# voitta-ai/voitta-rag

Measured on AMD Instinct MI355X. Metric: chunks indexed/sec + p50 top-10 query latency @1M-chunk corpus, 1/8 MI355X, higher is better.
Workload: dtype f16 (f16 MFMA operands, f32 accumulate; softmax, LayerNorm statistics and pooling in f32; the residual stream between layers is stored as f16 (LayerNorm is applied inside the GEMM epilogues from f32 row sums); measured |1-cos| = 1.5e-6 vs the f64 oracle on THIS code path at this scale — 2300 sequenc

## Files before the change

voitta_rag_amd/csrc/encoder.hip:

```cpp

#include "engine_internal.h"

#include <map>
#include <tuple>

#include <algorithm>
#include <cmath>

namespace vr {

using f32x4 = __attribute__((ext_vector_type(4))) float;
using f32x16 = __attribute__((ext_vector_type(16))) float;

struct SplitWeight {
  _Float16* hi = nullptr;
  _Float16* lo = nullptr;
  float unscale = 1.0f;
};

struct LayerWeights {
  float *wqkv, *bqkv, *wo, *bo, *ln1g, *ln1b, *w1, *b1, *w2, *b2, *ln2g, *ln2b;
  SplitWeight s_qkv, s_o, s_1, s_2;
  SplitWeight s_qkv_f{}, s_1_f{};
  float *cs_qkv = nullptr, *c_qkv = nullptr, *cs_1 = nullptr, *c_1 = nullptr;
  SplitWeight s_qkv_p{}, s_1_p{};
  float *bqkv_p = nullptr, *b1_p = nullptr;
  SplitWeight s_1_fp{};
  float *cs_1_p = nullptr, *c_1_p = nullptr;
  float *qn = nullptr, *kn = nullptr;
};

constexpr int kMaxHeadStages = 4;
struct HeadStage {
  int kind, in_dim, out_dim, act;
  float eps;
  const float *w, *b;
};
struct HeadParams {
  int n_stages;
  HeadStage st[kMaxHeadStages];
};

struct Encoder {
  vr_bert_desc d{};
  float *word = nullptr, *pos = nullptr, *type = nullptr, *lng = nullptr, *lnb = nullptr;
  std::vector<LayerWeights> layers;
  std::vector<float*> owned;
  int64_t ws_tokens = 0;
  float *x = nullptr, *qkv = nullptr, *ctx = nullptr, *tmp = nullptr, *ffn = nullptr;
  float* xs = nullptr;
  float* lnstat = nullptr;
  float* lnpart = nullptr;
  float* glu = nullptr;
  float2* rope = nullptr;
  float2* rope_local = nullptr;
  float* bias = nullptr;
  int bias_radius = 0;
  float* slopes = nullptr;
  bool has_head = false;
  HeadParams head{};
  int out_dim = 0;
  DevArray<float> pooled;
  int causal = 0;
  int dh = 0, attn = 0, qk_norm = 0;
  int window_stream_from = 0;
  float* posidx = nullptr;
  bool fuse = true;
  DevArray<int32_t> ids, cu, seg;
  DevArray<int32_t> span_tok, span_seq;
  std::vector<int32_t> span_seq_host;
  DevArray<int32_t> sem_off, sem_start, sem_idx, sem_seq_chunks, sem_seq_base, sem_counter;
  DevArray<float> sem_sums, sem_dist, sem_rows;
  DevArray<float> out;
  float *pool_w = nullptr, *pool_b = nullptr, *cls_w = nullptr, *cls_b = nullptr;
  float *head_ln_g = nullptr, *head_ln_b = nullptr;
  DevArray<float> rows;
  DevArray<float> skinny_ws;
  struct GraphKey {
    int T, n_seq, max_len;
    const void *ids, *cu, *seg, *out;
    const void *span_tok = nullptr, *span_seq = nullptr;
    int n_spans = 0;
    const void* pooled = nullptr;
    bool operator<(const GraphKey& o) const {
      return std::tie(T, n_seq, max_len, ids, cu, seg, out, span_tok, span_seq, n_spans, pooled) <
             std::tie(o.T, o.n_seq, o.max_len, o.ids, o.cu, o.seg, o.out, o.span_tok, o.span_seq, o.n_spans, o.pooled);
    }
  };
  struct GraphEntry {
    int seen = 0;
    bool bad = false;
    hipGraphExec_t exec = nullptr;
  };
  std::map<GraphKey, GraphEntry> graphs;
};

static void invalidate_graphs(Encoder* enc) {
  for (auto& kv : enc->graphs)
    if (kv.second.exec) (void)hipGraphExecDestroy(kv.second.exec);
  enc->graphs.clear();
}


__device__ __forceinline__ float wave_sum(float v) {
#pragma unroll
  for (int off = 32; off >= 1; off >>= 1) v += __shfl_xor(v, off);
  return v;
}

constexpr int kMaxPairs = 8;

using half_t = _Float16;
using f16x8 = __attribute__((ext_vector_type(8))) _Float16;

__device__ __forceinline__ void split_f16(float v, half_t& hi, half_t& lo) {
  v = fminf(fmaxf(v, -65504.0f), 65504.0f);
  hi = static_cast<half_t>(v);
  lo = static_cast<half_t>(v - static_cast<float>(hi));
}
// ... 877 lines not shown
  for (int t = 0; t < kHeadTiles; ++t) {
    const int col = (wave + 4 * t) * 16 + r;
    if (col < ocols)
#pragma unroll
      for (int i = 0; i < 4; ++i)
        if (p0 + 4 * q + i < n) out[static_cast<int64_t>(p0 + 4 * q + i) * ostride + col] = act[t][i];
  }
}

static int head_lda(const HeadParams& hp) {
  int k = 0;
  for (int s = 0; s < hp.n_stages; ++s)
    if (hp.st[s].kind == VR_HEAD_DENSE) k = std::max(k, hp.st[s].in_dim);
  return k + 4;
}
static size_t head_lds_bytes(int lda) { return (64 + 16 * static_cast<size_t>(lda)) * sizeof(float); }
constexpr int kMaxHeadWidth = 1024;

static int out_width(const Encoder* enc) { return enc->has_head ? enc->out_dim : enc->d.hidden; }

__global__ __launch_bounds__(256) void gather_first_rows_kernel(const float4* __restrict__ src,
                                                                const int32_t* __restrict__ cu, int seq0,
                                                                int tok_base, int n, int T, int row_f4,
                                                                float4* __restrict__ dst) {
  const int lane = threadIdx.x & 63;
  const int i = blockIdx.x * 4 + (threadIdx.x >> 6);
  if (i >= n) return;
  const int t = min(cu[seq0 + i] - tok_base, T - 1);
  for (int c = lane; c < row_f4; c += 64) dst[static_cast<int64_t>(i) * row_f4 + c] = src[static_cast<int64_t>(t) * row_f4 + c];
}

__global__ __launch_bounds__(256) void gather_first_rows_ln_kernel(const float* __restrict__ pre,
                                                                   const float2* __restrict__ stat,
                                                                   const float* __restrict__ g,
                                                                   const float* __restrict__ b,
                                                                   const int32_t* __restrict__ cu, int seq0,
                                                                   int tok_base, int n, int T, int H,
                                                                   float* __restrict__ dst) {
  const int lane = threadIdx.x & 63;
  const int i = blockIdx.x * 4 + (threadIdx.x >> 6);
  if (i >= n) return;
  const int t = min(cu[seq0 + i] - tok_base, T - 1);
  const float2 st = stat[t];
  for (int c = lane; c < H; c += 64)
    dst[static_cast<int64_t>(i) * H + c] = ln_apply(pre[static_cast<int64_t>(t) * H + c], st.x, st.y, g[c], b[c]);
}

__global__ __launch_bounds__(256) void gather_first_rows_ln16_kernel(const half_t* __restrict__ pre,
                                                                     const float2* __restrict__ stat,
                                                                     const float* __restrict__ g,
                                                                     const float* __restrict__ b,
                                                                     const int32_t* __restrict__ cu, int seq0,
                                                                     int tok_base, int n, int T, int H,
                                                                     float* __restrict__ dst) {
  const int lane = threadIdx.x & 63;
  const int i = blockIdx.x * 4 + (threadIdx.x >> 6);
  if (i >= n) return;
  const int t = min(cu[seq0 + i] - tok_base, T - 1);
  const float2 st = stat[t];
  for (int c = lane; c < H; c += 64)
    dst[static_cast<int64_t>(i) * H + c] =
        ln_apply(static_cast<float>(pre[static_cast<int64_t>(t) * H + c]), st.x, st.y, g[c], b[c]);
}


__device__ __forceinline__ void load8(const float* p, float (&v)[8]) {
  const float4 a = *reinterpret_cast<const float4*>(p), b = *reinterpret_cast<const float4*>(p + 4);
  v[0] = a.x, v[1] = a.y, v[2] = a.z, v[3] = a.w, v[4] = b.x, v[5] = b.y, v[6] = b.z, v[7] = b.w;
}
__device__ __forceinline__ void load8(const half_t* p, float (&v)[8]) {
  const f16x8 h = *reinterpret_cast<const f16x8*>(p);
#pragma unroll
  for (int k = 0; k < 8; ++k) v[k] = static_cast<float>(h[k]);
}
__device__ __forceinline__ void store8(float* p, const float (&v)[8]) {
  *reinterpret_cast<float4*>(p) = make_float4(v[0], v[1], v[2], v[3]);
  *reinterpret_cast<float4*>(p + 4) = make_float4(v[4], v[5], v[6], v[7]);
}
__device__ __forceinline__ void store8(half_t* p, const float (&v)[8]) {
  f16x8 h;
#pragma unroll
  for (int k = 0; k < 8; ++k) h[k] = static_cast<half_t>(fminf(fmaxf(v[k], -65504.0f), 65504.0f));
  *reinterpret_cast<f16x8*>(p) = h;
}

template <typename T>
__global__ __launch_bounds__(256) void rope_kernel(T* __restrict__ qkv, const int32_t* __restrict__ pos, int Tn, int H,
                                                   int dh, const float2* __restrict__ table) {
  const int lane = threadIdx.x & 63;
  const int t = blockIdx.x * 4 + (threadIdx.x >> 6);
  if (t >= Tn) return;
  const int half = dh >> 1;
  const int groups = half >> 3;
  const int per_third = (H / dh) * groups;
  T* row = qkv + static_cast<int64_t>(t) * 3 * H;
  const float2* cs_row = table + static_cast<int64_t>(pos[t]) * (H >> 1);
  for (int c = lane; c < 2 * per_third; c += 64) {
    const int third = c >= per_third ? 1 : 0;
    const int w = c - third * per_third;
    const int head = w / groups, i8 = (w - head * groups) << 3;
    T* at = row + third * H + head * dh + i8;
    float a[8], b[8], cs0[8], cs1[8];
    load8(at, a);
    load8(at + half, b);
    load8(reinterpret_cast<const float*>(cs_row + i8), cs0);
    load8(reinterpret_cast<const float*>(cs_row + i8 + 4), cs1);
    float ra[8], rb[8];
#pragma unroll
    for (int k = 0; k < 8; ++k) {
      const float co = k < 4 ? cs0[2 * k] : cs1[2 * k - 8], si = k < 4 ? cs0[2 * k + 1] : cs1[2 * k - 7];
      ra[k] = a[k] * co - b[k] * si;
      rb[k] = b[k] * co + a[k] * si;
    }
    store8(at, ra);
    store8(at + half, rb);
// ... 2620 lines not shown
        mx = fmaxf(mx, __shfl_xor(mx, 16));
        mx = fmaxf(mx, __shfl_xor(mx, 32));
        const float m_raw = fmaxf(m[i], mx);
        const float m_new = WIN || CAUSAL ? softmax_base(m_raw) : m_raw;
        const float alpha = __builtin_amdgcn_exp2f(m[i] - m_new);
        float psum = 0.0f;
#pragma unroll
        for (int t = 0; t < 4; ++t)
#pragma unroll
          for (int r = 0; r < 4; ++r) {
            const float p = __builtin_amdgcn_exp2f(st[i][t][r] - m_new);
            psum += p;
            pb[i][t >> 1][(t & 1) * 4 + r] = static_cast<half_t>(p);
          }
        l[i] = l[i] * alpha + psum;
        m[i] = m_raw;
#pragma unroll
        for (int s = 0; s < NS; ++s) o[i][s] *= alpha;
      }
#pragma unroll
      for (int u = 0; u < 2; ++u)
#pragma unroll
        for (int s = 0; s < NS; ++s) {
          const half_t* vb = sV + (32 * u + 4 * g) * LDK + tr_row + ((2 * s + (tr_p >> 1)) ^ tr_sw) * 8 + tr_in;
          const s16x4 lo = __builtin_amdgcn_ds_read_tr16_b64_v4i16((__attribute__((address_space(3))) s16x4*)(vb));
          const s16x4 hi = __builtin_amdgcn_ds_read_tr16_b64_v4i16((__attribute__((address_space(3))) s16x4*)(vb + 16 * LDK));
          f16x8 vf;
          *reinterpret_cast<s16x4*>(&vf) = lo;
          *(reinterpret_cast<s16x4*>(&vf) + 1) = hi;
          o[0][s] = __builtin_amdgcn_mfma_f32_16x16x32_f16(vf, pb[0][u], o[0][s], 0, 0, 0);
          if (two) o[1][s] = __builtin_amdgcn_mfma_f32_16x16x32_f16(vf, pb[1][u], o[1][s], 0, 0, 0);
        }
    }
    if (more) write(kt + 64, kr, vr, att_tiles + 2 * (buf ^ 1) * TILE, att_tiles + (2 * (buf ^ 1) + 1) * TILE);
    __syncthreads();
  }
  if (!active) return;
#pragma unroll
  for (int i = 0; i < 2; ++i) {
    float li = l[i];
    li += __shfl_xor(li, 16);
    li += __shfl_xor(li, 32);
    const int q_tok = qw + 16 * i + qi;
    if (q_tok < len && (i == 0 || two)) {
      const float inv = 1.0f / li;
      const int64_t off = static_cast<int64_t>(t0 + q_tok) * H + head * DH + 4 * g;
#pragma unroll
      for (int s = 0; s < NS; ++s) {
        half_t h[4];
#pragma unroll
        for (int r = 0; r < 4; ++r) h[r] = static_cast<half_t>(fminf(fmaxf(o[i][s][r] * inv, -65504.0f), 65504.0f));
        *reinterpret_cast<uint2*>(ctx_h + off + 16 * s) = *reinterpret_cast<const uint2*>(h);
      }
    }
  }
}


static int dev_alloc_copy(vr_engine* e, Encoder* enc, const void* src, size_t n_floats, int mem, float** out) {
  float* p = nullptr;
  VR_HIP(hipMalloc(reinterpret_cast<void**>(&p), n_floats * sizeof(float)));
  enc->owned.push_back(p);
  if (src)
    VR_HIP(hipMemcpyAsync(p, src, n_floats * sizeof(float),
                          mem == VR_MEM_HOST ? hipMemcpyHostToDevice : hipMemcpyDeviceToDevice, e->stream));
  *out = p;
  return 0;
}

__global__ void ln_finalize_kernel(const float2* __restrict__ part, int T, int segs, int H, float eps,
                                   float2* __restrict__ stat) {
  const int t = blockIdx.x * blockDim.x + threadIdx.x;
  if (t >= T) return;
  float s1 = 0.0f, s2 = 0.0f;
  for (int i = 0; i < segs; ++i) {
    const float2 p = part[static_cast<int64_t>(t) * segs + i];
    s1 += p.x;
    s2 += p.y;
  }
  const float mean = s1 / static_cast<float>(H);
  const float var = fmaxf(s2 / static_cast<float>(H) - mean * mean, 0.0f);
  stat[t] = make_float2(mean, 1.0f / sqrtf(var + eps));
}

__global__ void scale_cols_kernel(const float* __restrict__ w, const float* __restrict__ g, int64_t n, int K,
                                  float* __restrict__ out) {
  const int64_t i = static_cast<int64_t>(blockIdx.x) * blockDim.x + threadIdx.x;
  if (i < n) out[i] = w[i] * g[i % K];
}

__global__ __launch_bounds__(256) void fold_vectors_kernel(const half_t* __restrict__ wq, float unscale,
                                                           const float* __restrict__ w, const float* __restrict__ b,
                                                           const float* __restrict__ bias, int N, int K,
                                                           float* __restrict__ colsum, float* __restrict__ c) {
  const int lane = threadIdx.x & 63;
  const int n = blockIdx.x * 4 + (threadIdx.x >> 6);
  if (n >= N) return;
  double sq = 0.0, sc = 0.0;
  for (int k = lane; k < K; k += 64) {
    sq += static_cast<double>(static_cast<float>(wq[static_cast<int64_t>(n) * K + k]));
    sc += static_cast<double>(w[static_cast<int64_t>(n) * K + k]) * static_cast<double>(b[k]);
  }
#pragma unroll
  for (int off = 32; off >= 1; off >>= 1) {
    sq += __shfl_xor(sq, off);
    sc += __shfl_xor(sc, off);
// ... 139 lines not shown
           "position table are not implemented", d->position);
  VR_CHECK(!prenorm || gated, "norm VR_NORM_PRE needs a gated ffn (ffn %d): pre-norm encoders with the plain GELU "
           "feed-forward block are not implemented", d->ffn);
  VR_CHECK(d->window >= 0 && d->window <= 4096, "window %d must lie in 0..4096", d->window);
  VR_CHECK(d->window == 0 || rotary, "window %d needs position VR_POS_ROTARY (position %d)", d->window, d->position);
  VR_CHECK(d->window == 0 || prenorm, "window %d needs norm VR_NORM_PRE (norm %d): sliding-window attention in a "
           "post-norm encoder is not implemented", d->window, d->norm);
  VR_CHECK(d->window == 0 || d->global_every >= 1, "global_every %d must be >= 1 when window is set", d->global_every);
  VR_CHECK(d->rope_theta_local == 0.0f || (rotary && std::isfinite(d->rope_theta_local) && d->rope_theta_local > 0.0f),
           "rope_theta_local %g must be positive (or 0: rope_theta) and needs position VR_POS_ROTARY",
           static_cast<double>(d->rope_theta_local));
  VR_CHECK(d->max_pos >= 1 && d->max_pos <= 8192, "max_pos %d must lie in 1..8192 (the longest sequence the engine runs)",
           d->max_pos);
  VR_CHECK(L >= 1 && H >= 128 && H % 128 == 0 && H <= 1024, "hidden %d must be a multiple of 128 in 128..1024", H);
  VR_CHECK(I % 128 == 0 && I % BK == 0, "intermediate %d must be a multiple of 128", I);
  if (head_dim == 0)
    VR_CHECK(d->heads >= 1 && H % d->heads == 0 && (H / d->heads == 32 || H / d->heads == 64),
             "head size %d unsupported (32 or 64)", d->heads ? H / d->heads : 0);
  VR_CHECK(d->heads >= 1, "heads %d must be >= 1", d->heads);
  const int dh = head_dim ? head_dim : H / d->heads;
  const int64_t A64 = static_cast<int64_t>(d->heads) * dh;
  VR_CHECK(A64 % 128 == 0 && A64 <= 2048, "heads %d x head_dim %d = %lld: the attention width must be a multiple of 128 and at "
           "most 2048", d->heads, dh, static_cast<long long>(A64));
  const int A = static_cast<int>(A64);
  VR_CHECK(n_tensors == 5 + per_layer * L, "expected %d tensors, got %d", 5 + per_layer * L, n_tensors);
  VR_CHECK(d->pooling == VR_POOL_MEAN || d->pooling == VR_POOL_CLS || d->pooling == VR_POOL_LAST,
           "pooling %d must be 0 (mean), 1 (cls) or 2 (last token)", d->pooling);
  VR_CHECK(d->precision == VR_PRECISION_F32 || d->precision == VR_PRECISION_F16X3 || d->precision == VR_PRECISION_F16,
           "unknown precision %d", d->precision);
  for (int i = 0; i < n_tensors; ++i) {
    const int in_layer = i < 5 ? -1 : (i - 5) % per_layer;
    const bool bias = in_layer == 1 || in_layer == 3 || in_layer == 5 || in_layer == 7 || in_layer == 11 ||
                      in_layer == 13 || in_layer == 17;
    const bool rms_unused = (rms || rms_rot) && (i == 2 || i == 4 || in_layer == 9 || in_layer == 15);
    VR_CHECK(t[i] != nullptr || bias || rms_unused || (i == 1 && d->position != VR_POS_LEARNED), "tensor %d is null", i);
  }
  int window_stream_from = kWindowStreamFrom;
  if (const char* from = getenv("VR_WINDOW_STREAM_FROM")) {
    char* end = nullptr;
    const long v = strtol(from, &end, 10);
    VR_CHECK(end != from && *end == '\0' && v >= 1 && v <= INT32_MAX, "VR_WINDOW_STREAM_FROM='%s' must be a whole number >= 1",
             from);
    window_stream_from = static_cast<int>(v);
  }
  free_encoder(slot);
  Encoder* enc = new Encoder();
  *slot = enc;
  enc->d = *d;
  enc->causal = causal;
  enc->dh = dh;
  enc->attn = A;
  enc->qk_norm = qk_norm;
  enc->fuse = !(getenv("VR_ENCODE_FUSE") && atoi(getenv("VR_ENCODE_FUSE")) == 0);
  const size_t HH = static_cast<size_t>(A) * H;
  VR_TRY(dev_alloc_copy(e, enc, t[0], static_cast<size_t>(d->vocab) * H, mem, &enc->word));
  if (d->position == VR_POS_LEARNED) VR_TRY(dev_alloc_copy(e, enc, t[1], static_cast<size_t>(d->max_pos) * H, mem, &enc->pos));
  std::vector<float2> rope_host[2];
  auto rope_table = [&](float theta, std::vector<float2>& host, float2** out) -> int {
    const int half = dh / 2, row = A / 2;
    host.resize(static_cast<size_t>(d->max_pos) * row);
    for (int i = 0; i < half; ++i) {
      const double inv_freq = std::pow(static_cast<double>(theta), -2.0 * i / (2.0 * half));
      for (int p = 0; p < d->max_pos; ++p) {
        const double a = p * inv_freq;
        const float2 cs = make_float2(static_cast<float>(std::cos(a)), static_cast<float>(std::sin(a)));
        for (int h = 0; h < d->heads; ++h) host[static_cast<size_t>(p) * row + h * half + i] = cs;
      }
    }
    float* table = nullptr;
    VR_TRY(dev_alloc_copy(e, enc, host.data(), host.size() * 2, VR_MEM_HOST, &table));
    *out = reinterpret_cast<float2*>(table);
    return 0;
  };
  if (rotary) VR_TRY(rope_table(d->rope_theta, rope_host[0], &enc->rope));
  if (rotary && d->window > 0 && d->rope_theta_local != 0.0f && d->rope_theta_local != d->rope_theta)
    VR_TRY(rope_table(d->rope_theta_local, rope_host[1], &enc->rope_local));
  enc->window_stream_from = window_stream_from;
  if (rms || rms_rot) VR_TRY(dev_alloc_copy_or_zero(e, enc, t[2], H, mem, &enc->type));
  else VR_TRY(dev_alloc_copy(e, enc, t[2], static_cast<size_t>(d->type_vocab) * H, mem, &enc->type));
  VR_TRY(dev_alloc_copy(e, enc, t[3], H, mem, &enc->lng));
  if (!rms && !rms_rot) VR_TRY(dev_alloc_copy(e, enc, t[4], H, mem, &enc->lnb));
  const hipMemcpyKind kind = mem == VR_MEM_HOST ? hipMemcpyHostToDevice : hipMemcpyDeviceToDevice;
  for (int l = 0; l < L; ++l) {
    const void* const* w = t + 5 + per_layer * l;
    const int N1 = gated ? 2 * I : I;
    LayerWeights lw{};
    VR_TRY(dev_alloc_copy(e, enc, nullptr, 3 * HH, mem, &lw.wqkv));
    VR_TRY(dev_alloc_copy(e, enc, nullptr, 3 * static_cast<size_t>(A), mem, &lw.bqkv));
    for (int p = 0; p < 3; ++p) {
      VR_HIP(hipMemcpyAsync(lw.wqkv + p * HH, w[2 * p], HH * sizeof(float), kind, e->stream));
      if (w[2 * p + 1]) VR_HIP(hipMemcpyAsync(lw.bqkv + p * A, w[2 * p + 1], A * sizeof(float), kind, e->stream));
      else VR_HIP(hipMemsetAsync(lw.bqkv + p * A, 0, A * sizeof(float), e->stream));
    }
    if (qk_norm) {
      VR_TRY(dev_alloc_copy(e, enc, w[18], dh, mem, &lw.qn));
      VR_TRY(dev_alloc_copy(e, enc, w[19], dh, mem, &lw.kn));
    }
    VR_TRY(dev_alloc_copy(e, enc, w[6], HH, mem, &lw.wo));
    VR_TRY(dev_alloc_copy_or_zero(e, enc, w[7], H, mem, &lw.bo));
    VR_TRY(dev_alloc_copy(e, enc, w[8], H, mem, &lw.ln1g));
    if (!rms && !rms_rot) VR_TRY(dev_alloc_copy(e, enc, w[9], H, mem, &lw.ln1b));
    if (gated) {
      const size_t IH = static_cast<size_t>(I) * H;
      VR_TRY(dev_alloc_copy(e, enc, nullptr, 2 * IH, mem, &lw.w1));
      VR_TRY(dev_alloc_copy(e, enc, nullptr, 2 * static_cast<size_t>(I), mem, &lw.b1));
      for (int p = 0; p < 2; ++p) {
// ... 18 lines not shown
      VR_TRY(make_split(e, enc, lw.w1, static_cast<size_t>(N1) * H, H, plain, &lw.s_1));
      VR_TRY(make_split(e, enc, lw.w2, static_cast<size_t>(I) * H, I, plain, &lw.s_2));
      if (plain && (rotary || gated) && enc->fuse) {
        auto reordered = [&](const float* w_dev, const float* b_dev, int rows, int mode, int n, SplitWeight* sw, float** bias) -> int {
          const size_t cnt = static_cast<size_t>(rows) * H;
          float* tmp = nullptr;
          VR_HIP(hipMalloc(reinterpret_cast<void**>(&tmp), cnt * sizeof(float)));
          hipLaunchKernelGGL(reorder_rows_kernel, dim3(static_cast<unsigned>((cnt + 255) / 256)), dim3(256), 0, e->stream, w_dev,
                             static_cast<int64_t>(cnt), H, mode, n, H / d->heads, tmp);
          int rc = make_split(e, enc, tmp, cnt, H, true, sw);
          if (rc == 0) rc = dev_alloc_copy(e, enc, nullptr, rows, 0, bias);
          if (rc == 0)
            hipLaunchKernelGGL(reorder_rows_kernel, dim3(static_cast<unsigned>((rows + 255) / 256)), dim3(256), 0, e->stream, b_dev,
                               static_cast<int64_t>(rows), 1, mode, n, H / d->heads, *bias);
          (void)hipStreamSynchronize(e->stream);
          (void)hipFree(tmp);
          return rc;
        };
        if (rotary && !qk_norm && A == H) VR_TRY(reordered(lw.wqkv, lw.bqkv, 3 * H, 0, H, &lw.s_qkv_p, &lw.bqkv_p));
        if (gated) VR_TRY(reordered(lw.w1, lw.b1, 2 * I, 1, I, &lw.s_1_p, &lw.b1_p));
      }
      if (plain && H % 64 == 0 && !prenorm && !rms && !rms_rot) {
        auto fold = [&](const float* w_dev, int N, const float* g, const float* b, const float* bias, SplitWeight* sw,
                        float** colsum, float** c) -> int {
          const size_t n = static_cast<size_t>(N) * H;
          float* scaled = nullptr;
          VR_HIP(hipMalloc(reinterpret_cast<void**>(&scaled), n * sizeof(float)));
          hipLaunchKernelGGL(scale_cols_kernel, dim3(static_cast<unsigned>((n + 255) / 256)), dim3(256), 0, e->stream, w_dev,
                             g, static_cast<int64_t>(n), H, scaled);
          int rc = make_split(e, enc, scaled, n, H, true, sw);
          if (rc == 0) rc = dev_alloc_copy(e, enc, nullptr, N, 0, colsum);
          if (rc == 0) rc = dev_alloc_copy(e, enc, nullptr, N, 0, c);
          if (rc == 0)
            hipLaunchKernelGGL(fold_vectors_kernel, dim3(static_cast<unsigned>((N + 3) / 4)), dim3(256), 0, e->stream, sw->hi,
                               sw->unscale, w_dev, b, bias, N, H, *colsum, *c);
          (void)hipStreamSynchronize(e->stream);
          (void)hipFree(scaled);
          return rc;
        };
        VR_TRY(fold(lw.w1, N1, lw.ln1g, lw.ln1b, lw.b1, &lw.s_1_f, &lw.cs_1, &lw.c_1));
        if (gated && lw.b1_p) {
          const size_t cnt = static_cast<size_t>(N1) * H;
          float* inter = nullptr;
          VR_HIP(hipMalloc(reinterpret_cast<void**>(&inter), cnt * sizeof(float)));
          hipLaunchKernelGGL(reorder_rows_kernel, dim3(static_cast<unsigned>((cnt + 255) / 256)), dim3(256), 0, e->stream, lw.w1,
                             static_cast<int64_t>(cnt), H, 1, I, H / d->heads, inter);
          const int rc = fold(inter, N1, lw.ln1g, lw.ln1b, lw.b1_p, &lw.s_1_fp, &lw.cs_1_p, &lw.c_1_p);
          (void)hipFree(inter);
          VR_TRY(rc);
        }
        if (!enc->layers.empty()) {
          const LayerWeights& prev = enc->layers.back();
          VR_TRY(fold(lw.wqkv, 3 * H, prev.ln2g, prev.ln2b, lw.bqkv, &lw.s_qkv_f, &lw.cs_qkv, &lw.c_qkv));
        }
      }
    }
    enc->layers.push_back(lw);
  }
  VR_HIP(hipStreamSynchronize(e->stream));
  return 0;
}

int encoder_load(vr_engine* e, const vr_bert_desc* d, const void* const* t, int n_tensors, int mem) {
  return build_encoder(e, &e->encoder, d, t, n_tensors, mem);
}

int encoder_set_attention_bias(vr_engine* e, const float* table, int heads, int radius, int mem) {
  Encoder* enc = static_cast<Encoder*>(e->encoder);
  VR_CHECK(enc, "no encoder loaded");
  float* fresh = nullptr;
  if (table) {
    VR_CHECK((enc->d.position == VR_POS_LEARNED && enc->d.norm == VR_NORM_POST) ||
                 (enc->d.position == VR_POS_NONE && enc->d.norm == VR_NORM_PRE_RMS),
             "an attention bias needs position VR_POS_LEARNED and norm VR_NORM_POST (position %d, norm %d)", enc->d.position,
             enc->d.norm);
    VR_CHECK(heads == enc->d.heads, "bias table of %d heads for an encoder of %d", heads, enc->d.heads);
    VR_CHECK(!enc->slopes, "the encoder has attention slopes (vr_encoder_set_attention_slopes): remove them before a "
             "bias table is set");
    VR_CHECK(radius >= 1 && radius <= kMaxBiasRadius, "radius %d must lie in 1..%d", radius, kMaxBiasRadius);
    const size_t n = static_cast<size_t>(heads) * (2 * static_cast<size_t>(radius) + 1);
    VR_HIP(hipMalloc(reinterpret_cast<void**>(&fresh), n * sizeof(float)));
    hipError_t err = hipMemcpyAsync(fresh, table, n * sizeof(float),
                                    mem == VR_MEM_HOST ? hipMemcpyHostToDevice : hipMemcpyDeviceToDevice, e->stream);
    if (err == hipSuccess) err = hipStreamSynchronize(e->stream);
    if (err != hipSuccess) {
      (void)hipFree(fresh);
      VR_HIP(err);
    }
  } else {
    VR_HIP(hipStreamSynchronize(e->stream));
  }
  invalidate_graphs(enc);
  if (enc->bias) {
    enc->owned.erase(std::remove(enc->owned.begin(), enc->owned.end(), enc->bias), enc->owned.end());
    (void)hipFree(enc->bias);
  }
  enc->bias = fresh;
  enc->bias_radius = fresh ? radius : 0;
  if (fresh) enc->owned.push_back(fresh);
  return 0;
}

int encoder_set_attention_slopes(vr_engine* e, const float* slopes, int heads, int mem) {
  Encoder* enc = static_cast<Encoder*>(e->encoder);
  VR_CHECK(enc, "no encoder loaded");
  float* fresh = nullptr;
// ... 772 lines not shown
                       lnfuse ? nullptr : enc->x, xh, xl, lnfuse ? enc->x : nullptr, lnfuse ? stat_b : nullptr, seg_dev);
  else if (d.position != VR_POS_LEARNED)
    hipLaunchKernelGGL(embed_ln_rotary_kernel, dim3(row_blocks), dim3(256), 0, s, ids_dev, cu_dev, n_seq_total,
                       tok_base, T, H, d.vocab, enc->word, enc->type, enc->lng, enc->lnb, d.eps, lnfuse ? nullptr : enc->x, xh, xl,
                       lnfuse ? enc->x : nullptr, lnfuse ? stat_b : nullptr);
  else
    hipLaunchKernelGGL((embed_ln_kernel<false>), dim3(row_blocks), dim3(256), 0, s, ids_dev, cu_dev, n_seq_total,
                       tok_base, T, H, d.vocab, enc->word, enc->pos, enc->type, enc->lng, enc->lnb, d.eps,
                       lnfuse ? nullptr : enc->x, xh, xl, lnfuse ? enc->x : nullptr, lnfuse ? stat_b : nullptr,
                       static_cast<const int32_t*>(nullptr));
  const bool rotary = d.position == VR_POS_ROTARY, gated = d.ffn != VR_FFN_GELU;
  const int N1 = gated ? 2 * I : I;
  half_t* gluh = reinterpret_cast<half_t*>(enc->glu);
  const bool fuse_enabled = enc->fuse;
  const bool fuse_rope = rotary && plain && fuse_enabled && skinny_routed(T, 3 * H, H);
  auto fuse_glu = [&](int M) { return gated && plain && fuse_enabled && skinny_routed(M, N1, H); };
  const int glu_epi = d.ffn == VR_FFN_SWIGLU ? EPI_SWIGLU_F16 : EPI_GEGLU_F16;
  const bool fuse_glu_big = gated && fuse_enabled && !fuse_glu(T) && fold_big && pp_usable(N1, H) &&
                            enc->layers[0].cs_1_p != nullptr;
  const int32_t* posidx = reinterpret_cast<const int32_t*>(enc->posidx);
  half_t* qkvh = reinterpret_cast<half_t*>(enc->qkv);
  half_t* parth = reinterpret_cast<half_t*>(part);
  if (rotary)
    hipLaunchKernelGGL(positions_kernel, dim3(static_cast<unsigned>((T + 255) / 256)), dim3(256), 0, s, cu_dev, n_seq_total,
                       tok_base, T, reinterpret_cast<int32_t*>(enc->posidx));
  auto rope = [&]() {
    if (!rotary || fuse_rope) return;
    if (plain)
      hipLaunchKernelGGL(rope_kernel<half_t>, dim3(row_blocks), dim3(256), 0, s, reinterpret_cast<half_t*>(enc->qkv), posidx, T,
                         H, dh, enc->rope);
    else
      hipLaunchKernelGGL(rope_kernel<float>, dim3(row_blocks), dim3(256), 0, s, enc->qkv, posidx, T, H, dh, enc->rope);
  };
  auto glu = [&](int M, float* out, half_t* out_h) {
    const int64_t n8 = static_cast<int64_t>(M) * (I / 8);
    const dim3 grid(static_cast<unsigned>((n8 + 255) / 256));
    if (plain) hipLaunchKernelGGL((glu_kernel<half_t, 2>), grid, dim3(256), 0, s, gluh, n8, I, d.ffn, static_cast<float*>(nullptr), out_h);
    else if (split) hipLaunchKernelGGL((glu_kernel<float, 1>), grid, dim3(256), 0, s, enc->glu, n8, I, d.ffn, static_cast<float*>(nullptr), out_h);
    else hipLaunchKernelGGL((glu_kernel<float, 0>), grid, dim3(256), 0, s, enc->glu, n8, I, d.ffn, out, static_cast<half_t*>(nullptr));
  };
  const int n_seq = seq1 - seq0;
  const bool cls_tail = !sp && d.pooling == VR_POOL_CLS && !enc->layers.empty() &&
                        static_cast<int64_t>(n_seq) * (4 * H + I) <= static_cast<int64_t>(T) * 3 * H;
  if (gated && !enc->glu && ((!fuse_glu(T) && !fuse_glu_big) || (cls_tail && !fuse_glu(n_seq)))) {
    const size_t rows = static_cast<size_t>(enc->ws_tokens);
    VR_TRY(dev_alloc_copy(e, enc, nullptr, plain ? rows * I : rows * 2 * I, 0, &enc->glu));
    gluh = reinterpret_cast<half_t*>(enc->glu);
  }
  float* xc = enc->qkv;
  float* tmpc = xc + static_cast<int64_t>(n_seq) * H;
  float* xsc = tmpc + static_cast<int64_t>(n_seq) * H;
  float* ctxc = xsc + static_cast<int64_t>(n_seq) * H;
  float* ffnc = ctxc + static_cast<int64_t>(n_seq) * H;
  for (size_t li = 0; li < enc->layers.size(); ++li) {
    const LayerWeights& w = enc->layers[li];
    const bool tail = cls_tail && li + 1 == enc->layers.size();
    if (plain && fold_ln && li > 0 && fuse_rope)
      VR_TRY(launch_skinny_ln(e, EPI_ROPE_F16, cur.pre, d.eps, const_cast<float2*>(cur.stat),
                              {.W = w.s_qkv_p, .bias = w.bqkv_p, .Ch = qkvh, .M = T, .N = 3 * H, .K = H, .ln_g = cur.g,
                               .ln_b = cur.b, .rope_tab = enc->rope, .rope_pos = posidx}));
    else if (plain && fold_ln && li > 0)
      VR_TRY(launch_skinny_ln(e, EPI_BIAS_F16, cur.pre, d.eps, const_cast<float2*>(cur.stat),
                              {.W = w.s_qkv, .bias = w.bqkv, .Ch = qkvh, .M = T, .N = 3 * H, .K = H, .ln_g = cur.g, .ln_b = cur.b}));
    else if (plain && fold_big && li > 0)
      VR_TRY(launch_gemm_f16x3(e, enc, EPI_FOLD_F16, {.A = xh, .W = w.s_qkv_f, .bias = w.c_qkv, .Ch = qkvh, .M = T, .N = 3 * H,
                                                      .K = H, .passes = 1, .ln_stat = cur.stat, .ln_g = w.cs_qkv}));
    else if (plain && fuse_rope)
      VR_TRY(launch_gemm_f16x3(e, enc, EPI_ROPE_F16, {.A = xh, .W = w.s_qkv_p, .bias = w.bqkv_p, .Ch = qkvh, .M = T, .N = 3 * H,
                                                      .K = H, .passes = 1, .rope_tab = enc->rope, .rope_pos = posidx}));
    else if (plain)
      VR_TRY(launch_gemm_f16x3(e, enc, EPI_BIAS_F16, {.A = xh, .A_lo = xl, .W = w.s_qkv, .bias = w.bqkv, .Ch = qkvh, .M = T,
                                                      .N = 3 * H, .K = H, .passes = passes}));
    else if (split)
      VR_TRY(launch_gemm_f16x3(e, enc, EPI_BIAS, {.A = xh, .A_lo = xl, .W = w.s_qkv, .bias = w.bqkv, .C = enc->qkv, .M = T,
                                                  .N = 3 * H, .K = H, .passes = passes}));
    else
      VR_TRY(launch_gemm(e, EPI_BIAS, enc->x, w.wqkv, w.bqkv, nullptr, enc->qkv, T, 3 * H, H));
    rope();
    VR_TRY(launch_attention(e, enc, cu_dev, seq0, n_seq, tok_base, max_len, tail, 0, attn_flop));
    if (tail) {
      const unsigned gblocks = static_cast<unsigned>((n_seq + 3) / 4);
      const unsigned cblocks = gblocks;
      hipLaunchKernelGGL(gather_first_rows_kernel, dim3(gblocks), dim3(256), 0, s, reinterpret_cast<const float4*>(enc->ctx),
                         cu_dev, seq0, tok_base, n_seq, T, plain ? H / 8 : H / 4, reinterpret_cast<float4*>(ctxc));
      if (plain && cur16)
        hipLaunchKernelGGL(gather_first_rows_ln16_kernel, dim3(gblocks), dim3(256), 0, s, xh, cur.stat, cur.g, cur.b,
                           cu_dev, seq0, tok_base, n_seq, T, H, xc);
      else if (plain)
        hipLaunchKernelGGL(gather_first_rows_ln_kernel, dim3(gblocks), dim3(256), 0, s, cur.pre, cur.stat, cur.g, cur.b,
                           cu_dev, seq0, tok_base, n_seq, T, H, xc);
      else
        hipLaunchKernelGGL(gather_first_rows_kernel, dim3(gblocks), dim3(256), 0, s, reinterpret_cast<const float4*>(enc->x),
                           cu_dev, seq0, tok_base, n_seq, T, H / 4, reinterpret_cast<float4*>(xc));
      half_t* xch = reinterpret_cast<half_t*>(xsc);
      half_t* cch = reinterpret_cast<half_t*>(ctxc);
      half_t* fch = reinterpret_cast<half_t*>(ffnc);
      if (split)
        VR_TRY(launch_gemm_f16x3(e, enc, EPI_BIAS_RESIDUAL, {.A = cch, .A_lo = plain ? nullptr : cch + 8, .W = w.s_o, .bias = w.bo,
                                                             .R = xc, .C = tmpc, .M = n_seq, .N = H, .K = H, .passes = passes}));
      else
        VR_TRY(launch_gemm(e, EPI_BIAS_RESIDUAL, ctxc, w.wo, w.bo, xc, tmpc, n_seq, H, H));
      hipLaunchKernelGGL(layernorm_kernel, dim3(cblocks), dim3(256), 0, s, tmpc, n_seq, H, w.ln1g, w.ln1b, d.eps, xc,
                         split ? xch : nullptr, split && !plain ? xch + 8 : nullptr, static_cast<float2*>(nullptr));
      if (gated && fuse_glu(n_seq)) {
        VR_TRY(launch_gemm_f16x3(e, enc, glu_epi, {.A = xch, .W = w.s_1_p, .bias = w.b1_p, .Ch = fch, .M = n_seq, .N = N1, .K = H,
                                                   .passes = 1}));
      } else if (gated) {
        if (plain)
          VR_TRY(launch_gemm_f16x3(e, enc, EPI_BIAS_F16, {.A = xch, .W = w.s_1, .bias = w.b1, .Ch = gluh, .M = n_seq, .N = N1, .K = H,
                                                          .passes = 1}));
        else if (split)
          VR_TRY(launch_gemm_f16x3(e, enc, EPI_BIAS, {.A = xch, .A_lo = xch + 8, .W = w.s_1, .bias = w.b1, .C = enc->glu, .M = n_seq,
                                                      .N = N1, .K = H, .passes = passes}));
        else
          VR_TRY(launch_gemm(e, EPI_BIAS, xc, w.w1, w.b1, nullptr, enc->glu, n_seq, N1, H));
        glu(n_seq, ffnc, fch);
      } else if (split) {
        VR_TRY(launch_gemm_f16x3(e, enc, EPI_BIAS_GELU, {.A = xch, .A_lo = plain ? nullptr : xch + 8, .W = w.s_1, .bias = w.b1, .Ch = fch,
                                                         .Cl = plain ? nullptr : fch + 8, .M = n_seq, .N = I, .K = H, .passes = passes}));
      } else {
        VR_TRY(launch_gemm(e, EPI_BIAS_GELU, xc, w.w1, w.b1, nullptr, ffnc, n_seq, I, H));
      }
      if (split) {
        VR_TRY(launch_gemm_f16x3(e, enc, EPI_BIAS_RESIDUAL, {.A = fch, .A_lo = plain ? nullptr : fch + 8, .W = w.s_2, .bias = w.b2,
                                                             .R = xc, .C = tmpc, .M = n_seq, .N = H, .K = I, .passes = passes}));
      } else {
        VR_TRY(launch_gemm(e, EPI_BIAS_RESIDUAL, ffnc, w.w2, w.b2, xc, tmpc, n_seq, H, I));
      }
      hipLaunchKernelGGL(layernorm_kernel, dim3(cblocks), dim3(256), 0, s, tmpc, n_seq, H, w.ln2g, w.ln2b, d.eps, xc,
                         static_cast<half_t*>(nullptr), static_cast<half_t*>(nullptr), static_cast<float2*>(nullptr));
      launch_pool(e, enc, xc, cu_dev, seq0, seq1, tok_base, 1, out_dev, nullptr);
      VR_HIP(hipGetLastError());
      return 0;
    }
    if (plain) {
      float* t1 = cur.pre == enc->x ? enc->tmp : enc->x;
      float2* s1 = cur.stat == stat_b ? stat_a : stat_b;
      const bool last = li + 1 == enc->layers.size();
      if (res16) {
        VR_TRY(launch_gemm_f16x3(e, enc, cur16 ? EPI_RLS_R16_O16 : EPI_RLS_R32_O16,
// ... 431 lines not shown
```

Before: 48170.

## Collapse last-layer CLS attention by folding K and V projections into per-head algebra

For CLS pooling, the last layer now skips the full QKV GEMM over all tokens and the full attention. It computes Q only for the CLS rows and multiplies it by the transposed K weight to get a per-head vector U. It then scores tokens directly against the normalized hidden states using the LayerNorm stats, and projects the attention-weighted hidden states through the V weight afterwards. This removes the T×3H projection and the T-length attention in the final layer, at the cost of new custom kernels, a one-time weight transpose, and extra f16 rounding of the intermediate vectors.

New measurement: 48940, median of 6. 1.02x the previous value.

```diff
diff --git a/voitta_rag_amd/csrc/encoder.hip b/voitta_rag_amd/csrc/encoder.hip
--- a/voitta_rag_amd/csrc/encoder.hip
+++ b/voitta_rag_amd/csrc/encoder.hip
@@ -28,6 +28,7 @@
   SplitWeight s_1_fp{};
   float *cs_1_p = nullptr, *c_1_p = nullptr;
   float *qn = nullptr, *kn = nullptr;
+  _Float16* wk_t = nullptr;
 };
 
 constexpr int kMaxHeadStages = 4;
@@ -65,6 +66,7 @@
   int dh = 0, attn = 0, qk_norm = 0;
   int window_stream_from = 0;
   float* posidx = nullptr;
+  bool cls_collapse = true;
   bool fuse = true;
   DevArray<int32_t> ids, cu, seg;
   DevArray<int32_t> span_tok, span_seq;
@@ -1048,15 +1050,18 @@
                                                                      const float* __restrict__ b,
                                                                      const int32_t* __restrict__ cu, int seq0,
                                                                      int tok_base, int n, int T, int H,
-                                                                     float* __restrict__ dst) {
+                                                                     float* __restrict__ dst,
+                                                                     half_t* __restrict__ dst16) {
   const int lane = threadIdx.x & 63;
   const int i = blockIdx.x * 4 + (threadIdx.x >> 6);
   if (i >= n) return;
   const int t = min(cu[seq0 + i] - tok_base, T - 1);
   const float2 st = stat[t];
-  for (int c = lane; c < H; c += 64)
-    dst[static_cast<int64_t>(i) * H + c] =
-        ln_apply(static_cast<float>(pre[static_cast<int64_t>(t) * H + c]), st.x, st.y, g[c], b[c]);
+  for (int c = lane; c < H; c += 64) {
+    const float v = ln_apply(static_cast<float>(pre[static_cast<int64_t>(t) * H + c]), st.x, st.y, g[c], b[c]);
+    dst[static_cast<int64_t>(i) * H + c] = v;
+    if (dst16) dst16[static_cast<int64_t>(i) * H + c] = static_cast<half_t>(fminf(fmaxf(v, -65504.0f), 65504.0f));
+  }
 }
 
 
@@ -3783,6 +3788,200 @@
         for (int r = 0; r < 4; ++r) h[r] = static_cast<half_t>(fminf(fmaxf(o[i][s][r] * inv, -65504.0f), 65504.0f));
         *reinterpret_cast<uint2*>(ctx_h + off + 16 * s) = *reinterpret_cast<const uint2*>(h);
       }
+    }
+  }
+}
+
+constexpr int kClsHeads = 16;
+constexpr int kClsGroup = 16;
+constexpr int kClsStep = 32;
+using f16x4 = __attribute__((ext_vector_type(4))) _Float16;
+
+static size_t cls_attend_lds(int H, int lpad) {
+  return static_cast<size_t>(kClsHeads) * (static_cast<size_t>(std::max(H, lpad)) + 8) * sizeof(half_t) +
+         static_cast<size_t>(kClsHeads) * (static_cast<size_t>(lpad) + 4) * sizeof(float) + kClsHeads * sizeof(float);
+}
+
+__global__ void transpose_f16_kernel(const half_t* __restrict__ in, int H, half_t* __restrict__ out) {
+  const int64_t i = static_cast<int64_t>(blockIdx.x) * blockDim.x + threadIdx.x;
+  if (i >= static_cast<int64_t>(H) * H) return;
+  const int d = static_cast<int>(i / H), c = static_cast<int>(i % H);
+  out[i] = in[static_cast<int64_t>(c) * H + d];
+}
+
+template <bool CTX>
+__global__ __launch_bounds__(256) void cls_head_gemm_kernel(const half_t* __restrict__ W, int ldw, int64_t w_head,
+                                                            const half_t* __restrict__ A, int lda, int a_head, int M, int N,
+                                                            int K, float unscale, const float* __restrict__ cs,
+                                                            const float* __restrict__ c, const float* __restrict__ gamma,
+                                                            half_t* __restrict__ out, int ldo, int o_head) {
+  const int lane = threadIdx.x & 63;
+  const int wave = threadIdx.x >> 6;
+  const int head = blockIdx.z, nh = gridDim.z;
+  const int n0 = blockIdx.x * 64 + wave * 16;
+  const int row = lane & 15, g = lane >> 4;
+  const int m0 = blockIdx.y * 64;
+  if (n0 >= N) return;
+  const half_t* wp = W + head * w_head + static_cast<int64_t>(n0 + row) * ldw + 8 * g;
+  const half_t* ap[4];
+#pragma unroll
+  for (int mb = 0; mb < 4; ++mb)
+    ap[mb] = A + static_cast<int64_t>(min(m0 + mb * 16 + row, M - 1)) * lda + static_cast<int64_t>(head) * a_head + 8 * g;
+  f32x4 acc[4];
+#pragma unroll
+  for (int mb = 0; mb < 4; ++mb) acc[mb] = f32x4{0.f, 0.f, 0.f, 0.f};
+  const int mblocks = (min(M - m0, 64) + 15) / 16;
+  auto step = [&](int k) {
+    const f16x8 wf = *reinterpret_cast<const f16x8*>(wp + k);
+#pragma unroll
+    for (int mb = 0; mb < 4; ++mb)
+      if (mb < mblocks) {
+        const f16x8 af = *reinterpret_cast<const f16x8*>(ap[mb] + k);
+        acc[mb] = __builtin_amdgcn_mfma_f32_16x16x32_f16(wf, af, acc[mb], 0, 0, 0);
+      }
+  };
+  int k = 0;
+  for (; k + 64 <= K; k += 64) {
+    step(k);
+    step(k + 32);
+  }
+  if (k < K) step(k);
+  const int n = n0 + 4 * g;
+#pragma unroll
+  for (int mb = 0; mb < 4; ++mb) {
+    const int m = m0 + mb * 16 + row;
+    if (mb < mblocks && m < M) {
+      half_t h[4];
+#pragma unroll
+      for (int r = 0; r < 4; ++r) {
+        float v = acc[mb][r] * unscale;
+        if (CTX) {
+          const int col = head * N + n + r;
+          v = (v - cs[col] * gamma[static_cast<int64_t>(m) * nh + head]) + c[col];
+        }
+        h[r] = static_cast<half_t>(fminf(fmaxf(v, -65504.0f), 65504.0f));
+      }
+      *reinterpret_cast<uint2*>(out + static_cast<int64_t>(m) * ldo + static_cast<int64_t>(head) * o_head + n) =
+          *reinterpret_cast<const uint2*>(h);
+    }
+  }
+}
+
+__global__ __launch_bounds__(256) void cls_attend_kernel(const half_t* __restrict__ x, const float2* __restrict__ stat,
+                                                         const half_t* __restrict__ U, const int32_t* __restrict__ cu,
+                                                         int seq0, int tok_base, int T, int H, int nh, float scale2, int lpad,
+                                                         half_t* __restrict__ Z, float* __restrict__ gamma) {
+  extern __shared__ __align__(16) unsigned char cls_lds[];
+  const int tid = threadIdx.x, lane = tid & 63, wave = tid >> 6;
+  const int row = lane & 15, g = lane >> 4;
+  const int seq = blockIdx.x;
+  const int us = H + 8;
+  const int ps = lpad + 8;
+  const int ls = lpad + 4;
+  half_t* sU = reinterpret_cast<half_t*>(cls_lds);
+  half_t* sP = sU;
+  float* sS = reinterpret_cast<float*>(cls_lds + static_cast<size_t>(kClsHeads) * (max(H, lpad) + 8) * sizeof(half_t));
+  float* sA = sS + kClsHeads * ls;
+  const int t0 = cu[seq0 + seq] - tok_base;
+  const int len = min(min(cu[seq0 + seq + 1] - cu[seq0 + seq], T - t0), lpad);
+  half_t* zrow = Z + static_cast<int64_t>(seq) * nh * H;
+  if (len <= 0) {
+    for (int i = tid; i < nh * H; i += 256) zrow[i] = static_cast<half_t>(0.0f);
+    if (tid < nh) gamma[static_cast<int64_t>(seq) * nh + tid] = 0.0f;
+    return;
+  }
+  const int h8 = H >> 3;
+  for (int i = tid; i < kClsHeads * h8; i += 256) {
+    const int h = i / h8, c8 = i - h * h8;
+    f16x8 v = {0, 0, 0, 0, 0, 0, 0, 0};
+    if (h < nh) v = *reinterpret_cast<const f16x8*>(U + (static_cast<int64_t>(seq) * nh + h) * H + 8 * c8);
+    *reinterpret_cast<f16x8*>(sU + h * us + 8 * c8) = v;
+  }
+  __syncthreads();
+  for (int h = wave; h < kClsHeads; h += 4) {
+    float a = 0.0f;
+    for (int d = lane; d < H; d += 64) a += static_cast<float>(sU[h * us + d]);
+#pragma unroll
+    for (int off = 32; off >= 1; off >>= 1) a += __shfl_xor(a, off);
+    if (lane == 0) sA[h] = a;
+  }
+  __syncthreads();
+  const int groups = (len + kClsGroup - 1) / kClsGroup;
+  for (int gi = wave; gi < groups; gi += 4) {
+    const int tok = gi * kClsGroup + row;
+    const int tc = min(tok, len - 1);
+    const half_t* xp = x + static_cast<int64_t>(t0 + tc) * H + 8 * g;
+    const half_t* up = sU + row * us + 8 * g;
+    f32x4 acc = {0.f, 0.f, 0.f, 0.f};
+    for (int k = 0; k < H; k += 64) {
+      const f16x8 x0 = *reinterpret_cast<const f16x8*>(xp + k), x1 = *reinterpret_cast<const f16x8*>(xp + k + 32);
+      acc = __builtin_amdgcn_mfma_f32_16x16x32_f16(*reinterpret_cast<const f16x8*>(up + k), x0, acc, 0, 0, 0);
+      acc = __builtin_amdgcn_mfma_f32_16x16x32_f16(*reinterpret_cast<const f16x8*>(up + k + 32), x1, acc, 0, 0, 0);
+    }
+    const float2 st = stat[t0 + tc];
+    if (tok < len) {
+#pragma unroll
+      for (int r = 0; r < 4; ++r) sS[(4 * g + r) * ls + tok] = scale2 * st.y * (acc[r] - st.x * sA[4 * g + r]);
+    }
+  }
+  __syncthreads();
+  for (int h = wave; h < kClsHeads; h += 4) {
+    if (h >= nh) {
+      for (int j = lane; j < lpad; j += 64) sP[h * ps + j] = static_cast<half_t>(0.0f);
+      continue;
+    }
+    float m = -INFINITY;
+    for (int j = lane; j < len; j += 64) m = fmaxf(m, sS[h * ls + j]);
+#pragma unroll
+    for (int off = 32; off >= 1; off >>= 1) m = fmaxf(m, __shfl_xor(m, off));
+    float sum = 0.0f;
+    for (int j = lane; j < len; j += 64) sum += __builtin_amdgcn_exp2f(sS[h * ls + j] - m);
+#pragma unroll
+    for (int off = 32; off >= 1; off >>= 1) sum += __shfl_xor(sum, off);
+    const float inv_sum = 1.0f / sum;
+    float gm = 0.0f;
+    for (int j = lane; j < lpad; j += 64) {
+      half_t wh = static_cast<half_t>(0.0f);
+      if (j < len) {
+        const float2 st = stat[t0 + j];
+        wh = static_cast<half_t>(__builtin_amdgcn_exp2f(sS[h * ls + j] - m) * inv_sum * st.y);
+        gm += static_cast<float>(wh) * st.x;
+      }
+      sP[h * ps + j] = wh;
+    }
+#pragma unroll
+    for (int off = 32; off >= 1; off >>= 1) gm += __shfl_xor(gm, off);
+    if (lane == 0) gamma[static_cast<int64_t>(seq) * nh + h] = gm;
+  }
+  __syncthreads();
+  const half_t* pp = sP + row * ps + 8 * g;
+  for (int dg = wave; dg < (H >> 6); dg += 4) {
+    f32x4 acc[4];
+#pragma unroll
+    for (int q = 0; q < 4; ++q) acc[q] = f32x4{0.f, 0.f, 0.f, 0.f};
+    const half_t* xc = x + static_cast<int64_t>(t0) * H + 64 * dg + 4 * row;
+    for (int j0 = 0; j0 < lpad; j0 += kClsStep) {
+      f16x4 v[8];
+#pragma unroll
+      for (int i = 0; i < 8; ++i)
+        v[i] = *reinterpret_cast<const f16x4*>(xc + static_cast<int64_t>(min(j0 + 8 * g + i, len - 1)) * H);
+      const f16x8 pf = *reinterpret_cast<const f16x8*>(pp + j0);
+#pragma unroll
+      for (int q = 0; q < 4; ++q) {
+        const f16x8 xf = {v[0][q], v[1][q], v[2][q], v[3][q], v[4][q], v[5][q], v[6][q], v[7][q]};
+        acc[q] = __builtin_amdgcn_mfma_f32_16x16x32_f16(xf, pf, acc[q], 0, 0, 0);
+      }
+    }
+    if (row < nh) {
+      f16x8 o[2];
+#pragma unroll
+      for (int r = 0; r < 4; ++r)
+#pragma unroll
+        for (int q = 0; q < 4; ++q)
+          o[(4 * r + q) >> 3][(4 * r + q) & 7] = static_cast<half_t>(fminf(fmaxf(acc[q][r], -65504.0f), 65504.0f));
+      half_t* zp = zrow + static_cast<int64_t>(row) * H + 64 * dg + 16 * g;
+      *reinterpret_cast<f16x8*>(zp) = o[0];
+      *reinterpret_cast<f16x8*>(zp + 8) = o[1];
     }
   }
 }
@@ -4028,6 +4227,7 @@
   enc->attn = A;
   enc->qk_norm = qk_norm;
   enc->fuse = !(getenv("VR_ENCODE_FUSE") && atoi(getenv("VR_ENCODE_FUSE")) == 0);
+  enc->cls_collapse = slot == &e->encoder && !(getenv("VR_CLS_COLLAPSE") && atoi(getenv("VR_CLS_COLLAPSE")) == 0);
   const size_t HH = static_cast<size_t>(A) * H;
   VR_TRY(dev_alloc_copy(e, enc, t[0], static_cast<size_t>(d->vocab) * H, mem, &enc->word));
   if (d->position == VR_POS_LEARNED) VR_TRY(dev_alloc_copy(e, enc, t[1], static_cast<size_t>(d->max_pos) * H, mem, &enc->pos));
@@ -4152,6 +4352,14 @@
         if (!enc->layers.empty()) {
           const LayerWeights& prev = enc->layers.back();
           VR_TRY(fold(lw.wqkv, 3 * H, prev.ln2g, prev.ln2b, lw.bqkv, &lw.s_qkv_f, &lw.cs_qkv, &lw.c_qkv));
+          if (l + 1 == L && enc->cls_collapse && d->pooling == VR_POOL_CLS && A == H) {
+            float* kt = nullptr;
+            VR_TRY(dev_alloc_copy(e, enc, nullptr, HH / 2, 0, &kt));
+            lw.wk_t = reinterpret_cast<_Float16*>(kt);
+            hipLaunchKernelGGL(transpose_f16_kernel, dim3(static_cast<unsigned>((HH + 255) / 256)), dim3(256), 0, e->stream,
+                               lw.s_qkv_f.hi + HH, H, lw.wk_t);
+            VR_HIP(hipGetLastError());
+          }
         }
       }
     }
@@ -5030,10 +5238,47 @@
   float* xsc = tmpc + static_cast<int64_t>(n_seq) * H;
   float* ctxc = xsc + static_cast<int64_t>(n_seq) * H;
   float* ffnc = ctxc + static_cast<int64_t>(n_seq) * H;
+  const int cls_lpad = (max_len + kClsStep - 1) / kClsStep * kClsStep;
+  auto up4 = [](int64_t n) { return (n + 3) / 4 * 4; };
+  half_t* x16c = reinterpret_cast<half_t*>(ffnc + up4(static_cast<int64_t>(n_seq) * I));
+  half_t* q16c = x16c + up4(static_cast<int64_t>(n_seq) * H);
+  half_t* u16c = q16c + up4(static_cast<int64_t>(n_seq) * H);
+  half_t* z16c = u16c + up4(static_cast<int64_t>(n_seq) * nh * H);
+  float* gammac = reinterpret_cast<float*>(z16c + up4(static_cast<int64_t>(n_seq) * nh * H));
+  const int64_t cls_ws_floats = (gammac + static_cast<int64_t>(n_seq) * nh) - enc->qkv;
+  const bool collapse = cls_tail && enc->cls_collapse && plain && fold_big && res16 && enc->layers.size() > 1 &&
+                        enc->layers.back().wk_t != nullptr && d.position != VR_POS_ROTARY && !enc->bias && !enc->slopes &&
+                        !enc->causal && !enc->qk_norm && enc->attn == H && (dh == 32 || dh == 64) && nh <= kClsHeads &&
+                        cls_attend_lds(H, cls_lpad) <= 65536 && cls_ws_floats <= static_cast<int64_t>(T) * 3 * H;
   for (size_t li = 0; li < enc->layers.size(); ++li) {
     const LayerWeights& w = enc->layers[li];
     const bool tail = cls_tail && li + 1 == enc->layers.size();
-    if (plain && fold_ln && li > 0 && fuse_rope)
+    if (tail && collapse) {
+      const unsigned gblocks = static_cast<unsigned>((n_seq + 3) / 4);
+      const unsigned mblocks = static_cast<unsigned>((n_seq + 63) / 64);
+      hipLaunchKernelGGL(gather_first_rows_ln16_kernel, dim3(gblocks), dim3(256), 0, s, xh, cur.stat, cur.g, cur.b, cu_dev,
+                         seq0, tok_base, n_seq, T, H, xc, x16c);
+      VR_TRY(launch_gemm_f16x3(e, enc, EPI_BIAS_F16, {.A = x16c, .W = w.s_qkv, .bias = w.bqkv, .Ch = q16c, .M = n_seq, .N = H,
+                                                      .K = H, .passes = 1}));
+      const double head_flop = 2.0 * n_seq * static_cast<double>(H) * H;
+      prof_begin(e, VR_PROF_GEMM, head_flop);
+      hipLaunchKernelGGL((cls_head_gemm_kernel<false>), dim3(static_cast<unsigned>(H / 64), mblocks, static_cast<unsigned>(nh)),
+                         dim3(256), 0, s, w.wk_t, H, static_cast<int64_t>(dh), q16c, H, dh, n_seq, H, dh, w.s_qkv_f.unscale,
+                         static_cast<const float*>(nullptr), static_cast<const float*>(nullptr),
+                         static_cast<const float*>(nullptr), u16c, nh * H, H);
+      prof_end(e);
+      prof_begin(e, VR_PROF_ATTENTION, 4.0 * nh * static_cast<double>(H) * T);
+      hipLaunchKernelGGL(cls_attend_kernel, dim3(static_cast<unsigned>(n_seq)), dim3(256), cls_attend_lds(H, cls_lpad), s, xh,
+                         cur.stat, u16c, cu_dev, seq0, tok_base, T, H, nh, 1.4426950408889634f / sqrtf(static_cast<float>(dh)),
+                         cls_lpad, z16c, gammac);
+      prof_end(e);
+      prof_begin(e, VR_PROF_GEMM, head_flop);
+      hipLaunchKernelGGL((cls_head_gemm_kernel<true>), dim3(static_cast<unsigned>((dh + 63) / 64), mblocks, static_cast<unsigned>(nh)),
+                         dim3(256), 0, s, w.s_qkv_f.hi + static_cast<int64_t>(2) * H * H, H, static_cast<int64_t>(dh) * H, z16c,
+                         nh * H, H, n_seq, dh, H, w.s_qkv_f.unscale, w.cs_qkv + 2 * H, w.c_qkv + 2 * H, gammac,
+                         reinterpret_cast<half_t*>(ctxc), H, dh);
+      prof_end(e);
+    } else if (plain && fold_ln && li > 0 && fuse_rope)
       VR_TRY(launch_skinny_ln(e, EPI_ROPE_F16, cur.pre, d.eps, const_cast<float2*>(cur.stat),
                               {.W = w.s_qkv_p, .bias = w.bqkv_p, .Ch = qkvh, .M = T, .N = 3 * H, .K = H, .ln_g = cur.g,
                                .ln_b = cur.b, .rope_tab = enc->rope, .rope_pos = posidx}));
@@ -5054,16 +5299,21 @@
                                                   .N = 3 * H, .K = H, .passes = passes}));
     else
       VR_TRY(launch_gemm(e, EPI_BIAS, enc->x, w.wqkv, w.bqkv, nullptr, enc->qkv, T, 3 * H, H));
-    rope();
-    VR_TRY(launch_attention(e, enc, cu_dev, seq0, n_seq, tok_base, max_len, tail, 0, attn_flop));
+    if (!(tail && collapse)) {
+      rope();
+      VR_TRY(launch_attention(e, enc, cu_dev, seq0, n_seq, tok_base, max_len, tail, 0, attn_flop));
+    }
     if (tail) {
       const unsigned gblocks = static_cast<unsigned>((n_seq + 3) / 4);
       const unsigned cblocks = gblocks;
-      hipLaunchKernelGGL(gather_first_rows_kernel, dim3(gblocks), dim3(256), 0, s, reinterpret_cast<const float4*>(enc->ctx),
-                         cu_dev, seq0, tok_base, n_seq, T, plain ? H / 8 : H / 4, reinterpret_cast<float4*>(ctxc));
-      if (plain && cur16)
+      if (!collapse)
+        hipLaunchKernelGGL(gather_first_rows_kernel, dim3(gblocks), dim3(256), 0, s, reinterpret_cast<const float4*>(enc->ctx),
+                           cu_dev, seq0, tok_base, n_seq, T, plain ? H / 8 : H / 4, reinterpret_cast<float4*>(ctxc));
+      if (collapse)
+        ;
+      else if (plain && cur16)
         hipLaunchKernelGGL(gather_first_rows_ln16_kernel, dim3(gblocks), dim3(256), 0, s, xh, cur.stat, cur.g, cur.b,
-                           cu_dev, seq0, tok_base, n_seq, T, H, xc);
+                           cu_dev, seq0, tok_base, n_seq, T, H, xc, static_cast<half_t*>(nullptr));
       else if (plain)
         hipLaunchKernelGGL(gather_first_rows_ln_kernel, dim3(gblocks), dim3(256), 0, s, cur.pre, cur.stat, cur.g, cur.b,
                            cu_dev, seq0, tok_base, n_seq, T, H, xc);
```
